# jithendaraa/ODE-RL

Hardware: AMD Instinct MI355X
Metric: integrated latent frames/sec (ODEConvGRU, MovingMNIST) (higher is better)
Workload: dtype f32; 1 GPU; ODEConvGRU latents z0 (B=64,64,16,16) per GPU, T=10 output frames (9 intervals), fixed-step rk4 (3/8 rule), f = 5x conv3x3(64->64)+ReLU, forward only (BASELINE configs[1]); per_gpu_batch=64, frames=10, method=rk4, parallelism=batch-shard x1, nfe=36

## Files before the change

ode-rl_amd/csrc/conv_wino.hip:

```cpp
#include <stddef.h>
#include <stdlib.h>
#include <string.h>

#include "conv_common.h"

namespace odehip {

constexpr int kWU = 32 * 1024;
constexpr int kWRaw = 16 * 1024;
constexpr int kWV = 32 * 1024;
constexpr int kWinoLds = 2 * kWU + 2 * kWRaw + 2 * kWV;

__device__ __forceinline__ f32x4 pk_sub(f32x4 a, f32x4 b) {
  typedef float f32x2 __attribute__((ext_vector_type(2)));
  f32x2 lo, hi;
  const f32x2 alo = {a.x, a.y}, ahi = {a.z, a.w}, blo = {b.x, b.y}, bhi = {b.z, b.w};
  asm("v_pk_add_f32 %0, %1, %2 neg_lo:[0,1] neg_hi:[0,1]" : "=v"(lo) : "v"(alo), "v"(blo));
  asm("v_pk_add_f32 %0, %1, %2 neg_lo:[0,1] neg_hi:[0,1]" : "=v"(hi) : "v"(ahi), "v"(bhi));
  return f32x4{lo.x, lo.y, hi.x, hi.y};
}

struct PersistHook {
  unsigned* done = nullptr;
  unsigned target = 0u;
  int word0 = 0;
  unsigned* abort_ = nullptr;
  unsigned* host_err = nullptr;
  bool fence = false;
  float* nchw_base = nullptr;
  unsigned long long* stamps = nullptr;
  int batch = 0;
  bool first = true;
  bool solo = false;
  bool announce = true;
  bool split_wait = false;
  int sleep6 = 0;
  const unsigned long long* reloc = nullptr;
  unsigned wait_target = 0u;
};

template <typename T>
__device__ __forceinline__ T* rel(const unsigned long long* reloc, T* p) {
  const unsigned long long v = (unsigned long long)p;
  const unsigned cls = (unsigned)(v >> 56);
  if (cls == 0) return p;
  typedef const __attribute__((address_space(4))) unsigned long long ConstU;
  return (T*)((v & 0x00ffffffffffffffull) + *((ConstU*)reloc + cls));
}
__device__ __forceinline__ void pstamp(const PersistHook& hk, int i, int lane) {
  if (hk.stamps && lane == 0) hk.stamps[i] = __builtin_amdgcn_s_memrealtime();
}

template <typename T>
__device__ __forceinline__ T* uniform_ptr(T* p) {
  const unsigned long long v = (unsigned long long)p;
  const unsigned lo = __builtin_amdgcn_readfirstlane((unsigned)v), hi = __builtin_amdgcn_readfirstlane((unsigned)(v >> 32));
  return (T*)(((unsigned long long)hi << 32) | lo);
}

__device__ __forceinline__ void wait_done(const PersistHook& hk, int sel_mask = 0, int sel_val = 0) {
  int n = 0;
  const int lane = threadIdx.x & 63;
  const bool mine = lane < 16 && (lane & sel_mask) == sel_val;
  while (!__all(!mine || __hip_atomic_load(hk.done + (lane & 15), __ATOMIC_RELAXED, __HIP_MEMORY_SCOPE_AGENT) >= hk.wait_target)) {
    __builtin_amdgcn_s_sleep(1);
    if ((++n & 1023) == 0) {
      if (__hip_atomic_load(hk.abort_, __ATOMIC_RELAXED, __HIP_MEMORY_SCOPE_AGENT) == 1u) break;
      if (n > (1 << 23)) {
        __hip_atomic_store(hk.abort_, 1u, __ATOMIC_RELAXED, __HIP_MEMORY_SCOPE_AGENT);
        *hk.host_err = 3;
        break;
      }
    }
  }
  if (hk.fence) __builtin_amdgcn_fence(__ATOMIC_ACQUIRE, "agent");
}

__device__ __forceinline__ void announce(const PersistHook& hk, unsigned* done_word, bool stamp = false) {
  const int lane = threadIdx.x & 63;
  wait_vmcnt<0>();
  if (stamp) pstamp(hk, 7, lane);
  if (hk.fence) __builtin_amdgcn_fence(__ATOMIC_RELEASE, "agent");
  if (lane == 0 && hk.announce) __hip_atomic_store(done_word, hk.target + 1u, __ATOMIC_RELAXED, __HIP_MEMORY_SCOPE_AGENT);
}

template <int GROUP>
__device__ __forceinline__ bool xcc_rendezvous(unsigned* xcc_of, int lid, unsigned* abort_word, unsigned* host_err) {
  const unsigned my_xcc = (__builtin_amdgcn_s_getreg((3 << 11) | 20) & 15u) + 1u;
  if (threadIdx.x == 0) __hip_atomic_store(xcc_of + lid, my_xcc, __ATOMIC_RELAXED, __HIP_MEMORY_SCOPE_AGENT);
  bool fence = false;
  for (int p = 0; p < GROUP; ++p) {
    unsigned v = 0;
    int n = 0;
    while ((v = __hip_atomic_load(xcc_of + (lid & ~(GROUP - 1)) + p, __ATOMIC_RELAXED, __HIP_MEMORY_SCOPE_AGENT)) == 0) {
      __builtin_amdgcn_s_sleep(2);
      if (++n > (1 << 23)) {
        __hip_atomic_store(abort_word, 1u, __ATOMIC_RELAXED, __HIP_MEMORY_SCOPE_AGENT);
        *host_err = 2;
        break;
      }
    }
    fence |= (v != my_xcc);
  }
  return __builtin_amdgcn_readfirstlane(fence);
}

__device__ __forceinline__ bool walk_start(const ConvArgs*& table, int& n_layers, const int* section) {
  typedef const __attribute__((address_space(4))) int ConstI;
  const int* skip = table[0].skip;
  if (skip && *(ConstI*)skip) return false;
  if (section) {
    const int row0 = ((ConstI*)section)[0], n_dev = ((ConstI*)section)[1];
    if (row0 < 0 || n_dev <= 0 || row0 + n_dev > n_layers) return false;
    table += row0;
    n_layers = n_dev;
  }
  return true;
}

struct RowCursor {
  const ConvArgs* table;
  int n_layers;
  const float *src, *u, *src_next, *u_next;
  __device__ __forceinline__ RowCursor(const ConvArgs* t, int n)
      : table(t), n_layers(n), src(t[0].src1), u(t[0].w_wino), src_next(nullptr), u_next(nullptr) {}
  __device__ __forceinline__ const ConvArgs& row(int l) {
    typedef const __attribute__((address_space(4))) ConvArgs ConstArgs;
    const ConvArgs& a = *(const ConvArgs*)((ConstArgs*)table + l);
    src_next = src;
    u_next = u;
    if (l + 1 < n_layers) {
      src_next = table[l + 1].src1;
      u_next = table[l + 1].w_wino;
      if (threadIdx.x < (sizeof(ConvArgs) + 63) / 64) {
        const unsigned v = __builtin_nontemporal_load((const unsigned*)&table[l + 1] + threadIdx.x * 16);
        asm volatile("" ::"v"(v));
      }
    }
    return a;
  }
  __device__ __forceinline__ void next() {
    src = src_next;
    u = u_next;
  }
};

template <int NCHUNK, bool DBG, bool PERSIST, int QOUT = 16, bool ADAPT = false>
__device__ __forceinline__ void wino_layer(const float* __restrict__ p_src, const float* __restrict__ p_u, int p_qin, const ConvArgs& a,
                                           int b, int ct, int rh, char* smem, const PersistHook& hk) {
  static_assert(!PERSIST || (NCHUNK % 2 == 0), "the layer-to-layer LDS hand-over assumes an even chunk count");
  constexpr int kRawAux = PERSIST ? 16 : 0;
  char* const Ub = smem;
  char* const Rb = smem + 2 * kWU;
  char* const Vb = smem + 2 * kWU + 2 * kWRaw;
  Stamps st(a, (DBG && (a.debug & 16)) ? 256 : (DBG ? 0 : -1));
  st.take(0);
  const int tid = threadIdx.x;
  const int lane = tid & 63;
  const int wave = __builtin_amdgcn_readfirstlane(tid >> 6);
  const int r0 = rh * 8;
  constexpr int nchunk = NCHUNK;
  const bool skip = !PERSIST && a.skip && *a.skip;
  const bool dbg_noprod = DBG && (a.debug & 1), dbg_nomfma = DBG && (a.debug & 2), dbg_notr = DBG && (a.debug & 32),
             dbg_nodma = DBG && (a.debug & 128);

  if (wave >= 4) {
    const int pw = wave - 4, ptid = tid - 256;
    const unsigned u_tile_bytes = (unsigned)nchunk * kWU;
    const __amdgpu_buffer_rsrc_t ru = make_rsrc((const char*)p_u + (size_t)ct * u_tile_bytes, u_tile_bytes);
    const __amdgpu_buffer_rsrc_t rx = make_rsrc((const char*)p_src + (size_t)b * p_qin * kQuadBytes, (unsigned)p_qin * kQuadBytes);
    int vr[4];
#pragma unroll
    for (int p = 0; p < 4; ++p) {
      const int s = 64 * p + lane;
      const int row = s / 20, w = s - row * 20;
      const int pc = w < 9 ? 2 * w : 2 * (w - 9) + 1;
      const int irow = r0 - 1 + row, col = pc - 1;
      vr[p] = (s < 200 && w < 18 && irow >= 0 && irow < kHW && col >= 0 && col < kHW) ? irow * 256 + col * 16 : kOobOffset;
    }
    const int vw = lane * 16;
    auto issue_u = [&](int c, int buf) {
#pragma unroll
      for (int g = 0; g < 8; ++g) {
        const int p = pw * 8 + g;
        dma16(ru, Ub + buf * kWU + p * 1024, vw, (c * 32 + p) * 1024);
      }
    };
    auto issue_raw = [&](int c, int buf) {
#pragma unroll
      for (int p = 0; p < 4; ++p)
        __builtin_amdgcn_raw_ptr_buffer_load_lds(rx, ODEHIP_LDS_PTR(Rb + buf * kWRaw + (pw * 4 + p) * 1024), 16, vr[p],
                                                 (c * 4 + pw) * kQuadBytes, 0, kRawAux);
    };
    const int th = lane >> 5, tq = pw, tt = lane & 31;
    (void)ptid;
    const int tty = tt >> 3, ttx = tt & 7;
    const int r_a = th == 0 ? 2 : 1, r_b = th == 0 ? 0 : 2, r_c = th == 0 ? 1 : 3;
    const int raw_base = tq * 4096 + (2 * tty * 20 + ttx) * 16;
    const int off_a = raw_base + r_a * 320, off_b = raw_base + r_b * 320, off_c = raw_base + r_c * 320;
    const float sgn = th == 0 ? 1.0f : -1.0f;
    const int v_off = tq * 512 + tt * 16;
    auto transform = [&](int rbuf, int vbuf) {
      const char* r = Rb + rbuf * kWRaw;
      f32x4 d0[4], d1[4], d2[4];
#pragma unroll
      for (int j = 0; j < 4; ++j) {
        if (DBG && (a.debug & 512)) {
          d0[j] = d1[j] = d2[j] = f32x4{1.f, 2.f, 3.f, (float)j};
        } else {
          const int cj = ((j & 1) * 9 + (j >> 1)) * 16;
          d0[j] = *(const f32x4*)(r + off_a + cj);
          d1[j] = *(const f32x4*)(r + off_b + cj);
          d2[j] = *(const f32x4*)(r + off_c + cj);
        }
      }
      f32x4 T[2][4];
#pragma unroll
      for (int j = 0; j < 4; ++j) {
        T[0][j] = pk_sub(d1[j], d0[j]);
        T[1][j] = d2[j] + d0[j] * sgn;
      }
#pragma unroll
      for (int i = 0; i < 2; ++i) {
        char* v = Vb + vbuf * kWV + v_off + (2 * th + i) * 4 * 2048;
        if (DBG && (a.debug & 256)) {
          const f32x4 sum = (T[i][0] - T[i][2]) + (T[i][1] + T[i][2]) + (T[i][2] - T[i][1]) + (T[i][1] - T[i][3]);
          asm volatile("" ::"v"(sum.x), "v"(sum.y), "v"(sum.z), "v"(sum.w));
        } else {
          *(f32x4*)(v + 0 * 2048) = pk_sub(T[i][0], T[i][2]);
          *(f32x4*)(v + 1 * 2048) = T[i][1] + T[i][2];
          *(f32x4*)(v + 2 * 2048) = pk_sub(T[i][2], T[i][1]);
          *(f32x4*)(v + 3 * 2048) = pk_sub(T[i][1], T[i][3]);
        }
      }
    };

    if (PERSIST) {
      if (pw == 0) pstamp(hk, 0, lane);
      issue_u(0, 0);
      if (!hk.first) {
        if (hk.solo && hk.wait_target == hk.target)
          for (int i = 0; i < hk.sleep6; ++i) __builtin_amdgcn_s_sleep(6);
        if (hk.split_wait) wait_done(hk, 0x8, 0x0); else wait_done(hk);
      }
      if (pw == 0) pstamp(hk, 1, lane);
      issue_raw(0, 0);
      issue_raw(1, 1);
      wait_vmcnt<4>();
      if (pw == 0) pstamp(hk, 2, lane);
      transform(0, 0);
      if (pw == 0) pstamp(hk, 3, lane);
    } else if (!skip && !dbg_noprod) {
      issue_raw(0, 0);
      issue_u(0, 0);
      if (nchunk > 1) issue_raw(1, 1);
      if (nchunk > 1) wait_vmcnt<12>(); else wait_vmcnt<8>();
      transform(0, 0);
      if (nchunk > 1) wait_vmcnt<4>(); else wait_vmcnt<0>();
    }
    st.take(2);
#pragma unroll
    for (int c = 0; c < nchunk; ++c) {
      __builtin_amdgcn_s_barrier();
      if (!skip && !dbg_noprod && c + 1 < nchunk) {
        if (!dbg_nodma) issue_u(c + 1, (c + 1) & 1);
        if (c + 2 < nchunk) {
          if (PERSIST && c == 0 && !hk.first && hk.split_wait) wait_done(hk, 0x8, 0x8);
          if (!dbg_nodma) issue_raw(c + 2, c & 1);
          wait_vmcnt<12>();
        } else {
          wait_vmcnt<8>();
        }
        if (!dbg_notr) transform((c + 1) & 1, (c + 1) & 1);
        if (c + 2 < nchunk) wait_vmcnt<4>(); else wait_vmcnt<0>();
      }
      if (c < 4) st.take(3 + c);
    }
    st.flush(a);
    return;
  }

  const int ch = wave >> 1, thh = wave & 1;
  const int i16 = lane & 15, kq = lane >> 4;
  f32x4 acc[16];
#pragma unroll
  for (int x = 0; x < 16; ++x) acc[x] = f32x4{0.f, 0.f, 0.f, 0.f};
  const int u_off = kq * 512 + (ch * 16 + i16) * 16;
  const int v_off = kq * 512 + (thh * 16 + i16) * 16;
  const int Q = ct * 8 + ch * 4 + kq;
  f32x4 bias4 = {0.f, 0.f, 0.f, 0.f};
  if (a.bias) bias4 = *(const f32x4*)(a.bias + Q * 4);
  const int tile = thh * 16 + i16, oty = tile >> 3, otx = tile & 7;
  int e_combine = 0, e_act = 0, e_np = 0;
  float* e_dst = nullptr;
  float* e_kout = nullptr;
  float* e_out1 = nullptr;
  float* e_out2 = nullptr;
  float* e_nchw = nullptr;
  bool e_y = false;
  float e_h = 1.0f, e_ks = 1.0f, e_c1c = 0.0f, e_c2c = 0.0f, e_c1[3] = {0.f, 0.f, 0.f}, e_c2[3] = {0.f, 0.f, 0.f};
  f32x4 e_yv[4], e_kv[3][4];
  int d_kind = 0;
  f32x4 d_y[4], d_y1[4], d_sa[4], d_sb[4];
  float d_h = 1.0f, d_ks = 1.0f, d_cA = 0.0f, d_cB = 0.0f, d_rtol = 0.0f, d_atol = 0.0f, d_t[6] = {0.f, 0.f, 0.f, 0.f, 0.f, 0.f};
  float* d_o[4] = {nullptr, nullptr, nullptr, nullptr};
  bool d_has_y = false, d_err = false, d_f[4] = {false, false, false, false};
  if constexpr (ADAPT) {
    typedef const __attribute__((address_space(4))) float ConstF;
    const unsigned long long* const rl = hk.reloc;
    e_act = a.act;
    e_dst = rel(rl, a.dst);
    d_kind = a.combine == 0 ? 0 : 5;
    if (a.combine == 2) {
      const BwdArgs& w = a.bwd;
      const float hb = a.h_by_value ? a.cmb.atol : (w.h_ptr ? *(ConstF*)w.h_ptr : 0.0f);
      d_ks = w.sc_c + w.sc_h * hb;
      d_has_y = w.mask_src != nullptr;
      d_kind = 2;
      const float* const mask = rel(rl, w.mask_src);
#pragma unroll
      for (int q = 0; q < 4; ++q) {
        const size_t off = (((size_t)b * QOUT + Q) * kPix + (r0 + 2 * oty + (q >> 1)) * 16 + 2 * otx + (q & 1)) * 4;
        if (d_has_y) d_y[q] = *(const f32x4*)(mask + off);
      }
    } else if (a.combine == 3 && a.bwd.n_targets <= 2 && !a.bwd.h_ptr) {
      const BwdArgs& w = a.bwd;
      d_kind = 3;
#pragma unroll
      for (int t = 0; t < 2; ++t) {
        if (t < w.n_targets) {
          const BwdTarget& T = w.tgt[t];
          d_o[t] = rel(rl, T.out);
          d_t[3 * t] = T.g_c; d_t[3 * t + 1] = T.a_c; d_t[3 * t + 2] = T.b_c;
          d_f[2 * t] = T.srcA != nullptr; d_f[2 * t + 1] = T.srcB != nullptr;
          const float* const sA = rel(rl, T.srcA);
          const float* const sB = rel(rl, T.srcB);
#pragma unroll
          for (int q = 0; q < 4; ++q) {
            const size_t off = (((size_t)b * QOUT + Q) * kPix + (r0 + 2 * oty + (q >> 1)) * 16 + 2 * otx + (q & 1)) * 4;
            if (t == 0) {
              if (d_f[0]) d_y[q] = *(const f32x4*)(sA + off);
              if (d_f[1]) d_y1[q] = *(const f32x4*)(sB + off);
            } else {
              if (d_f[2]) d_sa[q] = *(const f32x4*)(sA + off);
              if (d_f[3]) d_sb[q] = *(const f32x4*)(sB + off);
            }
          }
        }
      }
    } else if (a.combine == 1 && (a.cmb.order == 1 || !a.cmb.y) && !(a.cmb.err_partials && (a.cmb.out2 || a.cmb.out2_nchw || a.dbg))) {
      const CombineArgs& m = a.cmb;
      d_kind = 1;
      const int np = m.n_prev;
      d_h = a.h_by_value ? m.atol : (m.h_ptr ? *(ConstF*)m.h_ptr : 1.0f);
      d_ks = m.k_scale;
      d_err = m.err_partials != nullptr;
      d_has_y = m.y != nullptr;
      d_cA = m.c1[np];
      d_cB = d_err ? m.ce[np] : m.c2[np];
      d_rtol = m.rtol; d_atol = m.atol;
      d_o[0] = rel(rl, m.k_out); d_o[1] = rel(rl, m.out1); d_o[2] = rel(rl, m.out2);
      d_o[3] = a.dbg ? hk.nchw_base + ((size_t)a.dbg - 1) : m.out2_nchw;
      const bool needB = d_err || d_o[2] || d_o[3];
      const float* const yp = rel(rl, m.y);
      const float* const y1p = rel(rl, m.err_y1);
#pragma unroll
      for (int q = 0; q < 4; ++q) {
        d_sa[q] = d_sb[q] = f32x4{0.f, 0.f, 0.f, 0.f};
        if (d_has_y) {
          const size_t off = (((size_t)b * QOUT + Q) * kPix + (r0 + 2 * oty + (q >> 1)) * 16 + 2 * otx + (q & 1)) * 4;
          d_y[q] = *(const f32x4*)(yp + off);
          if (d_err) d_y1[q] = *(const f32x4*)(y1p + off);
        }
      }
      if (d_has_y) {
        const float* kp[ODEHIP_MAX_STAGES - 1];
        float cA[ODEHIP_MAX_STAGES - 1], cB[ODEHIP_MAX_STAGES - 1];
#pragma unroll
        for (int j = 0; j < ODEHIP_MAX_STAGES - 1; ++j) {
          kp[j] = j < np ? rel(rl, m.k_prev[j]) : nullptr;
          cA[j] = m.c1[j];
          cB[j] = d_err ? m.ce[j] : m.c2[j];
        }
#pragma unroll
        for (int j = 0; j < ODEHIP_MAX_STAGES - 1; ++j) {
          if (j < np) {
#pragma unroll
            for (int q = 0; q < 4; ++q) {
              const size_t off = (((size_t)b * QOUT + Q) * kPix + (r0 + 2 * oty + (q >> 1)) * 16 + 2 * otx + (q & 1)) * 4;
              const f32x4 kv = *(const f32x4*)(kp[j] + off);
              d_sa[q] = fma4(kv, cA[j], d_sa[q]);
              if (needB) d_sb[q] = fma4(kv, cB[j], d_sb[q]);
            }
          }
        }
      }
    }
  } else if (PERSIST) {
    e_combine = a.combine;
    e_act = a.act;
    e_dst = a.dst;
    if (e_combine == 1 && !a.h_by_value) e_combine = 3;
    if (e_combine == 2) {
      const BwdArgs& w = a.bwd;
      typedef const __attribute__((address_space(4))) float ConstF;
      const float hb = a.h_by_value ? a.cmb.atol : (w.h_ptr ? *(ConstF*)w.h_ptr : 0.0f);
      e_ks = w.sc_c + w.sc_h * hb;
      e_y = w.mask_src != nullptr;
#pragma unroll
      for (int q = 0; q < 4; ++q) {
        const size_t off = (((size_t)b * QOUT + Q) * kPix + (r0 + 2 * oty + (q >> 1)) * 16 + 2 * otx + (q & 1)) * 4;
        if (e_y) e_yv[q] = *(const f32x4*)(w.mask_src + off);
      }
    } else if (e_combine == 1) {
      const CombineArgs& m = a.cmb;
      e_np = m.n_prev;
      e_h = m.atol;
      e_ks = m.k_scale;
      e_c1c = m.c1[e_np];
      e_c2c = m.c2[e_np];
      e_kout = m.k_out;
      e_out1 = m.out1;
      e_out2 = m.out2;
      e_nchw = a.dbg ? hk.nchw_base + ((size_t)a.dbg - 1) : nullptr;
      e_y = m.y != nullptr;
#pragma unroll
      for (int q = 0; q < 4; ++q) {
        const size_t off = (((size_t)b * QOUT + Q) * kPix + (r0 + 2 * oty + (q >> 1)) * 16 + 2 * otx + (q & 1)) * 4;
        if (e_y) e_yv[q] = *(const f32x4*)(m.y + off);
#pragma unroll
        for (int j = 0; j < 3; ++j)
          if (j < e_np) e_kv[j][q] = *(const f32x4*)(m.k_prev[j] + off);
      }
#pragma unroll
      for (int j = 0; j < 3; ++j) {
        e_c1[j] = m.c1[j];
        e_c2[j] = m.c2[j];
      }
    }
  }
  st.take(2);
#pragma unroll
  for (int c = 0; c < nchunk; ++c) {
    __builtin_amdgcn_s_barrier();
    if (PERSIST && c == 0 && wave == 0) pstamp(hk, 4, lane);
    if (!skip && !dbg_nomfma) {
      const char* u = Ub + (c & 1) * kWU + u_off;
      const char* v = Vb + (c & 1) * kWV + v_off;
      f32x4 w0 = *(const f32x4*)(u), x0 = *(const f32x4*)(v), w1 = *(const f32x4*)(u + 2048), x1 = *(const f32x4*)(v + 2048);
      f32x4 w0n, x0n, w1n, x1n;
#pragma unroll
      for (int x = 0; x < 16; x += 2) {
        if (x + 2 < 16) {
          w0n = *(const f32x4*)(u + (x + 2) * 2048);
          x0n = *(const f32x4*)(v + (x + 2) * 2048);
          w1n = *(const f32x4*)(u + (x + 3) * 2048);
          x1n = *(const f32x4*)(v + (x + 3) * 2048);
        }
        acc[x] = __builtin_amdgcn_mfma_f32_16x16x4f32(w0.x, x0.x, acc[x], 0, 0, 0);
        acc[x + 1] = __builtin_amdgcn_mfma_f32_16x16x4f32(w1.x, x1.x, acc[x + 1], 0, 0, 0);
        acc[x] = __builtin_amdgcn_mfma_f32_16x16x4f32(w0.y, x0.y, acc[x], 0, 0, 0);
        acc[x + 1] = __builtin_amdgcn_mfma_f32_16x16x4f32(w1.y, x1.y, acc[x + 1], 0, 0, 0);
        acc[x] = __builtin_amdgcn_mfma_f32_16x16x4f32(w0.z, x0.z, acc[x], 0, 0, 0);
        acc[x + 1] = __builtin_amdgcn_mfma_f32_16x16x4f32(w1.z, x1.z, acc[x + 1], 0, 0, 0);
        acc[x] = __builtin_amdgcn_mfma_f32_16x16x4f32(w0.w, x0.w, acc[x], 0, 0, 0);
        acc[x + 1] = __builtin_amdgcn_mfma_f32_16x16x4f32(w1.w, x1.w, acc[x + 1], 0, 0, 0);
        w0 = w0n; x0 = x0n; w1 = w1n; x1 = x1n;
        __builtin_amdgcn_sched_group_barrier(0x008, 1, 0);
        __builtin_amdgcn_sched_group_barrier(0x100, 4, 0);
        __builtin_amdgcn_sched_group_barrier(0x008, 7, 0);
        __builtin_amdgcn_sched_barrier(0);
      }
    }
    if (st.on && c < 4) {
      asm volatile("" ::"v"(acc[15][0]));
      st.take(3 + c);
    }
  }
  if (skip) return;
  if (PERSIST && wave == 0) pstamp(hk, 5, lane);

  f32x4 S[2][4];
#pragma unroll
  for (int cI = 0; cI < 4; ++cI) {
    S[0][cI] = acc[0 * 4 + cI] + acc[1 * 4 + cI] + acc[2 * 4 + cI];
    S[1][cI] = pk_sub(pk_sub(acc[1 * 4 + cI], acc[2 * 4 + cI]), acc[3 * 4 + cI]);
  }
  float esum = 0.0f;
  auto emit_pre = [&](int q, int P, f32x4 v) {
    const size_t off = (((size_t)b * QOUT + Q) * kPix + P) * 4;
    if (!e_combine) {
      *(f32x4*)(e_dst + off) = act_fwd(v, e_act);
      return;
    }
    if (e_combine == 2) {
      v *= e_ks;
      if (e_y) v = act_bwd(v, e_yv[q], e_act);
      *(f32x4*)(e_dst + off) = v;
      return;
    }
    if (e_combine == 3) {
      emit_quad<false>(a, b, Q, P, v, esum);
      return;
    }
    const f32x4 kc = act_fwd(v, e_act) * e_ks;
    if (e_kout) *(f32x4*)(e_kout + off) = kc;
    if (e_y) {
      if (e_out1) {
        f32x4 sa = kc * e_c1c;
#pragma unroll
        for (int j = 0; j < 3; ++j)
          if (j < e_np) sa += e_kv[j][q] * e_c1[j];
        *(f32x4*)(e_out1 + off) = e_yv[q] + sa * e_h;
      }
      if (e_out2 || e_nchw) {
        f32x4 sb = kc * e_c2c;
#pragma unroll
        for (int j = 0; j < 3; ++j)
          if (j < e_np) sb += e_kv[j][q] * e_c2[j];
        const f32x4 o2 = e_yv[q] + sb * e_h;
        if (e_out2) *(f32x4*)(e_out2 + off) = o2;
        if (e_nchw) {
          float* o = e_nchw + ((size_t)b * (QOUT * 4) + Q * 4) * kPix + P;
          o[0] = o2.x; o[kPix] = o2.y; o[2 * kPix] = o2.z; o[3 * kPix] = o2.w;
        }
      }
    }
  };
  auto emit_adapt = [&](int q, int P, f32x4 v) {
    const size_t off = (((size_t)b * QOUT + Q) * kPix + P) * 4;
    if (d_kind == 0) {
      *(f32x4*)(e_dst + off) = act_fwd(v, e_act);
    } else if (d_kind == 2) {
      v *= d_ks;
      if (d_has_y) v = act_bwd(v, d_y[q], e_act);
      *(f32x4*)(e_dst + off) = v;
    } else if (d_kind == 1) {
      const f32x4 kc = act_fwd(v, e_act) * d_ks;
      if (d_o[0]) *(f32x4*)(d_o[0] + off) = kc;
      if (d_has_y) {
        if (d_o[1]) *(f32x4*)(d_o[1] + off) = fma4(fma4(kc, d_cA, d_sa[q]), d_h, d_y[q]);
        if (d_err) {
          esum = combine1_err(fma4(kc, d_cB, d_sb[q]), d_h, d_y[q], d_y1[q], d_rtol, d_atol, esum);
        } else if (d_o[2] || d_o[3]) {
          const f32x4 o2 = fma4(fma4(kc, d_cB, d_sb[q]), d_h, d_y[q]);
          if (d_o[2]) *(f32x4*)(d_o[2] + off) = o2;
          if (d_o[3]) {
            float* o = d_o[3] + ((size_t)b * (QOUT * 4) + Q * 4) * kPix + P;
            o[0] = o2.x; o[kPix] = o2.y; o[2 * kPix] = o2.z; o[3 * kPix] = o2.w;
          }
        }
      }
    } else if (d_kind == 3) {
      if (d_o[0]) {
        f32x4 o = v * d_t[0];
        if (d_f[0]) o = fma4(d_y[q], d_t[1], o);
        if (d_f[1]) o = fma4(d_y1[q], d_t[2], o);
        *(f32x4*)(d_o[0] + off) = o;
      }
      if (d_o[1]) {
        f32x4 o = v * d_t[3];
        if (d_f[2]) o = fma4(d_sa[q], d_t[4], o);
        if (d_f[3]) o = fma4(d_sb[q], d_t[5], o);
        *(f32x4*)(d_o[1] + off) = o;
      }
    } else {
      emit_quad(a, b, Q, P, v, esum, a.dbg ? hk.nchw_base + ((size_t)a.dbg - 1) : nullptr);
    }
  };
#pragma unroll
  for (int i = 0; i < 2; ++i) {
    const f32x4 y0 = S[i][0] + S[i][1] + S[i][2] + bias4;
    const f32x4 y1 = pk_sub(pk_sub(S[i][1] + bias4, S[i][2]), S[i][3]);
    const int P = (r0 + 2 * oty + i) * 16 + 2 * otx;
    if constexpr (ADAPT) {
      emit_adapt(2 * i, P, y0);
      emit_adapt(2 * i + 1, P + 1, y1);
    } else if (PERSIST) {
      emit_pre(2 * i, P, y0);
      emit_pre(2 * i + 1, P + 1, y1);
    } else {
      emit_quad(a, b, Q, P, y0, esum);
      emit_quad(a, b, Q, P + 1, y1, esum);
    }
  }
  if (PERSIST) {
    if (a.combine == 1 && a.cmb.err_partials) {
#pragma unroll
      for (int o = 32; o > 0; o >>= 1) esum += __shfl_xor(esum, o, 64);
      const int nwg_pl = (QOUT / 4) * hk.batch, lid_pl = b * (QOUT / 4) + ct * 2 + rh;
      const int bid_pl = (nwg_pl & 7) == 0 ? (lid_pl % (nwg_pl >> 3)) * 8 + lid_pl / (nwg_pl >> 3) : lid_pl;
      if (lane == 0) a.cmb.err_partials[bid_pl * 4 + wave] = esum;
    }
    if (wave == 0) pstamp(hk, 6, lane);
    announce(hk, hk.done + hk.word0 + wave, wave == 0);
  } else {
    finish_err(a, esum, wave);
    st.flush(a);
  }
}

template <int NCHUNK, bool DBG>
__global__ __launch_bounds__(512, 1) void conv3x3_wino_kernel(const float* __restrict__ p_src, const float* __restrict__ p_u,
                                                              int p_qin, int p_qout, const ConvArgs a) {
  extern __shared__ __attribute__((aligned(16))) char smem[];
  (void)p_qout;
  const int nwg = gridDim.x * gridDim.y;
  int lid = blockIdx.x + gridDim.x * blockIdx.y;
  if ((nwg & 7) == 0) lid = (lid & 7) * (nwg >> 3) + (lid >> 3);
  const int rh = lid & 1, ct = (lid >> 1) % (gridDim.x >> 1), b = (lid >> 1) / (gridDim.x >> 1);
  const PersistHook none;
  wino_layer<NCHUNK, DBG, false>(p_src, p_u, p_qin, a, b, ct, rh, smem, none);
}

struct PersistArgs {
  const ConvArgs* table;
  int n_layers, batch;
  unsigned* done;
  unsigned* xcc_of;
  unsigned* host_err;
  float* out_nchw;
  unsigned long long* stamps;
  int sleep6;
  int sleep6_combine;
  const int* n_layers_ptr;
  const unsigned long long* reloc;
  int fault_inject;
};

template <int QOUT>
__device__ __forceinline__ void ew_row(const ConvArgs& a, int b, int ct, int rh, const PersistHook& hk) {
  const int tid = threadIdx.x, lane = tid & 63;
  const int wave = __builtin_amdgcn_readfirstlane(tid >> 6);
  if (wave >= 4) return;
  typedef const __attribute__((address_space(4))) float ConstF;
  const CombineArgs& m = a.cmb;
  const unsigned long long* const rl = hk.reloc;
  const float hs = m.h_ptr ? *(ConstF*)m.h_ptr : 1.0f;
  const int ch = wave >> 1, thh = wave & 1, i16 = lane & 15, kq = lane >> 4;
  const int Q = ct * 8 + ch * 4 + kq, tile = thh * 16 + i16, oty = tile >> 3, otx = tile & 7, r0 = rh * 8;
  const float* const yp = rel(rl, m.y);
  if (a.combine == 5) {
    const float* const pa = rel(rl, m.k_prev[0]);
    const float* const pb = m.n_prev > 1 ? rel(rl, m.k_prev[1]) : nullptr;
    float sum = 0.0f;
#pragma unroll
    for (int q = 0; q < 4; ++q) {
      const size_t o = (((size_t)b * QOUT + Q) * kPix + (r0 + 2 * oty + (q >> 1)) * 16 + 2 * otx + (q & 1)) * 4;
      f32x4 d = *(const f32x4*)(pa + o);
      const f32x4 yv = *(const f32x4*)(yp + o);
      if (pb) d -= *(const f32x4*)(pb + o);
#pragma unroll
      for (int i = 0; i < 4; ++i) {
        const float r = d[i] / __builtin_fmaf(fabsf(yv[i]), m.rtol, m.atol);
        sum = __builtin_fmaf(r, r, sum);
      }
    }
#pragma unroll
    for (int o = 32; o > 0; o >>= 1) sum += __shfl_xor(sum, o, 64);
    if (lane == 0) m.err_partials[(b * 4 + ct * 2 + rh) * 4 + wave] = sum;
    wait_vmcnt<0>();
    if (hk.fence) __builtin_amdgcn_fence(__ATOMIC_RELEASE, "agent");
    if (lane == 0) __hip_atomic_store(hk.done + hk.word0 + wave, hk.target + 1u, __ATOMIC_RELAXED, __HIP_MEMORY_SCOPE_AGENT);
    return;
  }
  float* const o1 = rel(rl, m.out1);
  float* const o2 = rel(rl, m.out2);
  f32x4 s1[4], s2[4];
  size_t off[4];
#pragma unroll
  for (int q = 0; q < 4; ++q) {
    off[q] = (((size_t)b * QOUT + Q) * kPix + (r0 + 2 * oty + (q >> 1)) * 16 + 2 * otx + (q & 1)) * 4;
    s1[q] = f32x4{0.f, 0.f, 0.f, 0.f};
    if (yp) s1[q] = *(const f32x4*)(yp + off[q]);
    s2[q] = s1[q];
  }
  for (int j = 0; j < m.n_prev; ++j) {
    const float* const kp = rel(rl, m.k_prev[j]);
    const float c1 = (m.c_dev ? ((ConstF*)m.c_dev)[j] : m.c1[j]) * hs;
    const float c2 = m.c2[j] * hs;
#pragma unroll
    for (int q = 0; q < 4; ++q) {
      const f32x4 kv = *(const f32x4*)(kp + off[q]);
      s1[q] = fma4(kv, c1, s1[q]);
      if (o2) s2[q] = fma4(kv, c2, s2[q]);
    }
  }
#pragma unroll
  for (int q = 0; q < 4; ++q) {
    if (o1) *(f32x4*)(o1 + off[q]) = s1[q];
    if (o2) *(f32x4*)(o2 + off[q]) = s2[q];
  }
  wait_vmcnt<0>();
  if (hk.fence) __builtin_amdgcn_fence(__ATOMIC_RELEASE, "agent");
  if (lane == 0) __hip_atomic_store(hk.done + hk.word0 + wave, hk.target + 1u, __ATOMIC_RELAXED, __HIP_MEMORY_SCOPE_AGENT);
}

template <bool ADAPT>
__device__ __forceinline__ void persist_walk(const PersistArgs& pa, const ConvArgs* table) {
  extern __shared__ __attribute__((aligned(16))) char smem[];
  const int nwg = gridDim.x;
  const int lid = ((int)blockIdx.x & 7) * (nwg >> 3) + ((int)blockIdx.x >> 3);
  const int rh = lid & 1, ct = (lid >> 1) & 1, group = lid >> 2;
  const bool fence = xcc_rendezvous<4>(pa.xcc_of, lid, pa.xcc_of + nwg, pa.host_err);
  int n_layers = pa.n_layers;
  if (!walk_start(table, n_layers, ADAPT ? pa.n_layers_ptr : nullptr)) return;
  const int n_groups = nwg >> 2;
  for (int b = group; b < pa.batch; b += 2 * n_groups) {
    const int n_interleaved = b + n_groups < pa.batch ? 2 : 1;
    RowCursor cur(table, n_layers);
    int prev_combine = 0;
    for (int l = 0; l < n_layers; ++l) {
      const ConvArgs& a = cur.row(l);
#pragma unroll 1
      for (int s = 0; s < n_interleaved; ++s) {
        const int bs = __builtin_amdgcn_readfirstlane(b + s * n_groups);
        const PersistHook hk = {pa.done + (size_t)bs * kDoneStride, (unsigned)l, (lid & 3) * 4, pa.xcc_of + nwg, pa.host_err, fence,
                                pa.out_nchw, (pa.stamps && lid == 0 && bs == group && l < 64) ? pa.stamps + l * 8 : nullptr, pa.batch,
                                l == 0, n_interleaved == 1, true, true, pa.sleep6 + (prev_combine == 1 ? pa.sleep6_combine : 0),
                                ADAPT ? pa.reloc : nullptr,
                                (unsigned)(ADAPT && a.dep_back > 0 && l > 0 ? l - 1 : l)};
        if constexpr (ADAPT) {
          if (a.combine >= 4) ew_row<16>(a, bs, ct, rh, hk);
          else wino_layer<4, false, true, 16, true>(uniform_ptr(rel(pa.reloc, cur.src)), uniform_ptr(cur.u), 16, a, bs, ct, rh, smem, hk);
        } else {
          wino_layer<4, false, true>(uniform_ptr(cur.src), uniform_ptr(cur.u), 16, a, bs, ct, rh, smem, hk);
        }
      }
      prev_combine = a.combine;
      cur.next();
    }
  }
}

__global__ __launch_bounds__(512, 1) void wino_persist_kernel(const PersistArgs pa) { persist_walk<false>(pa, pa.table); }

__global__ __launch_bounds__(512, 1) void wino_persist_d_kernel(const PersistArgs pa) { persist_walk<true>(pa, pa.table); }

__device__ __forceinline__ void persist_walk_v(const PersistArgs& pa, const ConvArgs* table) {
  extern __shared__ __attribute__((aligned(16))) char smem[];
  const int nwg = gridDim.x;
  const int lid = ((int)blockIdx.x & 7) * (nwg >> 3) + ((int)blockIdx.x >> 3);
  const int rh = lid & 1, ct = (lid >> 1) & 1, group = lid >> 2;
  const bool fence = xcc_rendezvous<4>(pa.xcc_of, lid, pa.xcc_of + nwg, pa.host_err);
  {
    typedef const __attribute__((address_space(4))) int ConstI;
    const int* skip = table[0].skip;
    if (skip && *(ConstI*)skip) return;
  }
  const int n_groups = nwg >> 2;
  for (int b = group; b < pa.batch; b += 2 * n_groups) {
    const int n_interleaved = b + n_groups < pa.batch ? 2 : 1;
    int prev_combine = 0;
    for (int l = 0; l < pa.n_layers; ++l) {
      typedef const __attribute__((address_space(4))) ConvArgs ConstArgs;
      const ConvArgs& a = *(const ConvArgs*)((ConstArgs*)table + l);
      if (l + 1 < pa.n_layers && threadIdx.x < (sizeof(ConvArgs) + 63) / 64) {
        const unsigned v = __builtin_nontemporal_load((const unsigned*)&table[l + 1] + threadIdx.x * 16);
        asm volatile("" ::"v"(v));
      }
      const float* src = uniform_ptr(a.src1);
      const float* u = uniform_ptr(a.w_wino);
      const int qin = a.qin, qout = a.qout;
#pragma unroll 1
      for (int s = 0; s < n_interleaved; ++s) {
        const int bs = __builtin_amdgcn_readfirstlane(b + s * n_groups);
        PersistHook hk = {pa.done + (size_t)bs * kDoneStride, (unsigned)l, (lid & 3) * 4, pa.xcc_of + nwg, pa.host_err, fence,
                          pa.out_nchw, nullptr, pa.batch, l == 0, n_interleaved == 1, true, false,
                          pa.sleep6 + (prev_combine == 1 ? pa.sleep6_combine : 0), nullptr, (unsigned)l};
        if (qout == 16) {
          if (qin == 16) wino_layer<4, false, true, 16>(src, u, 16, a, bs, ct, rh, smem, hk);
          else           wino_layer<8, false, true, 16>(src, u, 32, a, bs, ct, rh, smem, hk);
// ... 554 lines not shown
```

Before: 468,700 latent frames/s.

## Stream Winograd weights directly into MFMA wave registers instead of staging via LDS

Removes the double-buffered LDS staging of the transformed weights U, which producer waves previously DMA'd into shared memory. The MFMA waves now load U straight from global memory with buffer loads into an 8-entry register ring prefetched ahead of use. This frees 64 KB of LDS, possibly allowing more occupancy, and removes LDS read traffic and producer DMA work. In exchange the consumer waves take on global-load latency and extra VGPR pressure, and each wave redundantly fetches weights that were previously shared across waves.

After: 488,900 latent frames/s, median of 6. 1.04x the previous value.

```diff
diff --git a/ode-rl_amd/csrc/conv_wino.hip b/ode-rl_amd/csrc/conv_wino.hip
--- a/ode-rl_amd/csrc/conv_wino.hip
+++ b/ode-rl_amd/csrc/conv_wino.hip
@@ -9,7 +9,12 @@
 constexpr int kWU = 32 * 1024;
 constexpr int kWRaw = 16 * 1024;
 constexpr int kWV = 32 * 1024;
-constexpr int kWinoLds = 2 * kWU + 2 * kWRaw + 2 * kWV;
+constexpr int kWinoLds = 2 * kWRaw + 2 * kWV;
+constexpr int kUAhead = 8;
+
+__device__ __forceinline__ f32x4 load_u(__amdgpu_buffer_rsrc_t r, int voffset, int soffset) {
+  return __builtin_bit_cast(f32x4, __builtin_amdgcn_raw_buffer_load_b128(r, voffset, soffset, 0));
+}
 
 __device__ __forceinline__ f32x4 pk_sub(f32x4 a, f32x4 b) {
   typedef float f32x2 __attribute__((ext_vector_type(2)));
@@ -149,10 +154,10 @@
 __device__ __forceinline__ void wino_layer(const float* __restrict__ p_src, const float* __restrict__ p_u, int p_qin, const ConvArgs& a,
                                            int b, int ct, int rh, char* smem, const PersistHook& hk) {
   static_assert(!PERSIST || (NCHUNK % 2 == 0), "the layer-to-layer LDS hand-over assumes an even chunk count");
+  static_assert(kUAhead % 2 == 0 && kUAhead <= 16, "the U ring is refilled a pair of positions at a time");
   constexpr int kRawAux = PERSIST ? 16 : 0;
-  char* const Ub = smem;
-  char* const Rb = smem + 2 * kWU;
-  char* const Vb = smem + 2 * kWU + 2 * kWRaw;
+  char* const Rb = smem;
+  char* const Vb = smem + 2 * kWRaw;
   Stamps st(a, (DBG && (a.debug & 16)) ? 256 : (DBG ? 0 : -1));
   st.take(0);
   const int tid = threadIdx.x;
@@ -166,8 +171,6 @@
 
   if (wave >= 4) {
     const int pw = wave - 4, ptid = tid - 256;
-    const unsigned u_tile_bytes = (unsigned)nchunk * kWU;
-    const __amdgpu_buffer_rsrc_t ru = make_rsrc((const char*)p_u + (size_t)ct * u_tile_bytes, u_tile_bytes);
     const __amdgpu_buffer_rsrc_t rx = make_rsrc((const char*)p_src + (size_t)b * p_qin * kQuadBytes, (unsigned)p_qin * kQuadBytes);
     int vr[4];
 #pragma unroll
@@ -178,14 +181,6 @@
       const int irow = r0 - 1 + row, col = pc - 1;
       vr[p] = (s < 200 && w < 18 && irow >= 0 && irow < kHW && col >= 0 && col < kHW) ? irow * 256 + col * 16 : kOobOffset;
     }
-    const int vw = lane * 16;
-    auto issue_u = [&](int c, int buf) {
-#pragma unroll
-      for (int g = 0; g < 8; ++g) {
-        const int p = pw * 8 + g;
-        dma16(ru, Ub + buf * kWU + p * 1024, vw, (c * 32 + p) * 1024);
-      }
-    };
     auto issue_raw = [&](int c, int buf) {
 #pragma unroll
       for (int p = 0; p < 4; ++p)
@@ -237,7 +232,6 @@
 
     if (PERSIST) {
       if (pw == 0) pstamp(hk, 0, lane);
-      issue_u(0, 0);
       if (!hk.first) {
         if (hk.solo && hk.wait_target == hk.target)
           for (int i = 0; i < hk.sleep6; ++i) __builtin_amdgcn_s_sleep(6);
@@ -252,27 +246,23 @@
       if (pw == 0) pstamp(hk, 3, lane);
     } else if (!skip && !dbg_noprod) {
       issue_raw(0, 0);
-      issue_u(0, 0);
       if (nchunk > 1) issue_raw(1, 1);
-      if (nchunk > 1) wait_vmcnt<12>(); else wait_vmcnt<8>();
+      if (nchunk > 1) wait_vmcnt<4>(); else wait_vmcnt<0>();
       transform(0, 0);
-      if (nchunk > 1) wait_vmcnt<4>(); else wait_vmcnt<0>();
     }
     st.take(2);
 #pragma unroll
     for (int c = 0; c < nchunk; ++c) {
       __builtin_amdgcn_s_barrier();
       if (!skip && !dbg_noprod && c + 1 < nchunk) {
-        if (!dbg_nodma) issue_u(c + 1, (c + 1) & 1);
         if (c + 2 < nchunk) {
           if (PERSIST && c == 0 && !hk.first && hk.split_wait) wait_done(hk, 0x8, 0x8);
           if (!dbg_nodma) issue_raw(c + 2, c & 1);
-          wait_vmcnt<12>();
+          wait_vmcnt<4>();
         } else {
-          wait_vmcnt<8>();
+          wait_vmcnt<0>();
         }
         if (!dbg_notr) transform((c + 1) & 1, (c + 1) & 1);
-        if (c + 2 < nchunk) wait_vmcnt<4>(); else wait_vmcnt<0>();
       }
       if (c < 4) st.take(3 + c);
     }
@@ -287,6 +277,15 @@
   for (int x = 0; x < 16; ++x) acc[x] = f32x4{0.f, 0.f, 0.f, 0.f};
   const int u_off = kq * 512 + (ch * 16 + i16) * 16;
   const int v_off = kq * 512 + (thh * 16 + i16) * 16;
+  constexpr int kG = 16 * NCHUNK;
+  const bool dbg_nou = dbg_noprod || dbg_nodma;
+  const __amdgpu_buffer_rsrc_t ru = make_rsrc((const char*)p_u + (size_t)ct * (NCHUNK * kWU), (unsigned)NCHUNK * kWU);
+  f32x4 uw[kUAhead];
+#pragma unroll
+  for (int g = 0; g < kUAhead; ++g) {
+    if (skip || dbg_nou) uw[g] = f32x4{1.f, 1.f, 1.f, 1.f};
+    else uw[g] = load_u(ru, u_off, g * 2048);
+  }
   const int Q = ct * 8 + ch * 4 + kq;
   f32x4 bias4 = {0.f, 0.f, 0.f, 0.f};
   if (a.bias) bias4 = *(const f32x4*)(a.bias + Q * 4);
@@ -445,17 +444,20 @@
     __builtin_amdgcn_s_barrier();
     if (PERSIST && c == 0 && wave == 0) pstamp(hk, 4, lane);
     if (!skip && !dbg_nomfma) {
-      const char* u = Ub + (c & 1) * kWU + u_off;
       const char* v = Vb + (c & 1) * kWV + v_off;
-      f32x4 w0 = *(const f32x4*)(u), x0 = *(const f32x4*)(v), w1 = *(const f32x4*)(u + 2048), x1 = *(const f32x4*)(v + 2048);
-      f32x4 w0n, x0n, w1n, x1n;
+      f32x4 x0 = *(const f32x4*)(v), x1 = *(const f32x4*)(v + 2048);
+      f32x4 x0n, x1n;
 #pragma unroll
       for (int x = 0; x < 16; x += 2) {
+        const int g = c * 16 + x, s0 = g % kUAhead, s1 = (g + 1) % kUAhead;
+        const f32x4 w0 = uw[s0], w1 = uw[s1];
         if (x + 2 < 16) {
-          w0n = *(const f32x4*)(u + (x + 2) * 2048);
           x0n = *(const f32x4*)(v + (x + 2) * 2048);
-          w1n = *(const f32x4*)(u + (x + 3) * 2048);
           x1n = *(const f32x4*)(v + (x + 3) * 2048);
+        }
+        if (g + kUAhead < kG && !dbg_nou) {
+          uw[s0] = load_u(ru, u_off, (g + kUAhead) * 2048);
+          uw[s1] = load_u(ru, u_off, (g + kUAhead + 1) * 2048);
         }
         acc[x] = __builtin_amdgcn_mfma_f32_16x16x4f32(w0.x, x0.x, acc[x], 0, 0, 0);
         acc[x + 1] = __builtin_amdgcn_mfma_f32_16x16x4f32(w1.x, x1.x, acc[x + 1], 0, 0, 0);
@@ -465,9 +467,10 @@
         acc[x + 1] = __builtin_amdgcn_mfma_f32_16x16x4f32(w1.z, x1.z, acc[x + 1], 0, 0, 0);
         acc[x] = __builtin_amdgcn_mfma_f32_16x16x4f32(w0.w, x0.w, acc[x], 0, 0, 0);
         acc[x + 1] = __builtin_amdgcn_mfma_f32_16x16x4f32(w1.w, x1.w, acc[x + 1], 0, 0, 0);
-        w0 = w0n; x0 = x0n; w1 = w1n; x1 = x1n;
+        x0 = x0n; x1 = x1n;
         __builtin_amdgcn_sched_group_barrier(0x008, 1, 0);
-        __builtin_amdgcn_sched_group_barrier(0x100, 4, 0);
+        __builtin_amdgcn_sched_group_barrier(0x100, 2, 0);
+        __builtin_amdgcn_sched_group_barrier(0x020, 2, 0);
         __builtin_amdgcn_sched_group_barrier(0x008, 7, 0);
         __builtin_amdgcn_sched_barrier(0);
       }
```
